# MG-RAST/Shock

Hardware: AMD Instinct MI355X
Metric: device-resident index-build GiB/s + Mrecords/s, 10 GiB FASTQ, 1/2/4/8 GPU (higher is better)
Workload: dtype u8; 1 GPU; fastq record index, 10 GiB synthetic node file in HBM (BASELINE configs[1]); records=30969274, bytes=10737418240, tile=16384, parallelism=single slab, exchange=none (one slab: no collective)

## Files before the change

### shock_amd/csrc/sidx_build.cpp

```cpp
#include <errno.h>
#include <hip/hip_runtime.h>
#include <stdio.h>
#include <stdlib.h>
#include <string.h>
#include <sys/mman.h>
#include <unistd.h>

#include <atomic>
#include <mutex>
#include <vector>

#include "../../include/shockidx.h"
#include "sidx_common.hpp"
#include "sidx_subset.hpp"
#include "sidx_launch.hpp"
#include "sidx_host.hpp"

using namespace sidx;

namespace sidx_host {

CopyPool::CopyPool(int n) : nt_(n) {
  for (int i = 0; i < n; ++i) th_.emplace_back([this, i] { run(i); });
}
CopyPool::~CopyPool() {
  {
    std::lock_guard<std::mutex> g(m_);
    stop_ = true;
    ++gen_;
  }
  cv_.notify_all();
  for (auto &t : th_) t.join();
}
void CopyPool::copy(void *dst, const void *src, size_t n) {
  uint8_t *d = (uint8_t *)dst;
  const uint8_t *sp = (const uint8_t *)src;
  parallel(n, [d, sp](size_t a, size_t b) { memcpy(d + a, sp + a, b - a); });
}
void CopyPool::parallel(size_t n, const std::function<void(size_t, size_t)> &f) {
  if (n < (4u << 20) || nt_ < 2) {
    if (n) f(0, n);
    return;
  }
  std::unique_lock<std::mutex> lk(m_);
  fn_ = &f;
  n_ = n;
  pending_ = nt_;
  ++gen_;
  cv_.notify_all();
  done_.wait(lk, [this] { return pending_ == 0; });
}
void CopyPool::run(int i) {
  unsigned long long seen = 0;
// ... 172 lines not shown
  p.n = n;
  p.end = geom ? geom->end : n;
  p.front = geom ? geom->front : 0;
  p.base = geom ? geom->base : 0;
  p.state_in = geom ? geom->state_in : 0;
  p.row_base = geom ? geom->row_base : 0;
  p.summary = geom ? (u64 *)geom->d_summary : nullptr;
  p.row_cap = row_cap;
  p.rows = d_rows;
  auto status_array = [c](StatusArray a) { return c->d_status + (u64)a * c->tiles_cap(); };
  p.status = status_array(SA_STATUS);
  p.pcnt = status_array(SA_PCNT);
  p.ppre = status_array(SA_PPRE);
  for (int i = 0; i < 2; ++i) p.scan_look[i] = status_array((StatusArray)(SA_LOOK0 + i));
  p.tile_agg = status_array(SA_TILE_AGG);
  p.tile_excl = status_array(SA_TILE_EXCL);
  p.pgrid = c->tiles_grid < ntiles ? c->tiles_grid : (u32)ntiles;
  p.fix = general ? nullptr : c->d_fix.get();
  p.fixcap = (u32)c->tiles_cap();
  p.grid_cap = c->grid_cap;
  p.badkey = (u64 *)(c->d_small + SMALL_BADKEY + 8 * slot);
  p.badkey_next = (u64 *)(c->d_small + SMALL_BADKEY + 8 * (slot ^ 1));
  p.detail = c->d_detail;
  p.counters = (u32 *)(c->d_small + SMALL_COUNTERS + 4 * NCOUNTERS * slot);
  p.counters_next = (u32 *)(c->d_small + SMALL_COUNTERS + 4 * NCOUNTERS * (slot ^ 1));
  p.ntiles = (u32)ntiles;
  p.epoch = c->epoch;
  p.seq = geom ? geom->seq : 0;
  p.inject = (c->inject & 4) ? 1u : 0u;
  p.eof = geom ? geom->eof : 1;
  p.file_start = geom ? geom->file_start : 1;
  p.gate = gate;
  p.gate_fmt = kfmt;
  if (const char *dbg = getenv("SHOCKIDX_DEBUG")) p.debug = (u32)atoi(dbg);
  if (getenv("SHOCKIDX_TIMING")) {
    HIPCHK(hipMemsetAsync(c->d_timing, 0, 9 * 8 * 65536, s), "timing clear");
    p.timing = c->d_timing;
  }
  DevResult *d_res = (DevResult *)(c->d_small + SMALL_RESULT);
  const bool tile_pass = pass != TP_TWO_PASS;
  if (tile_pass) {
    p.tile_stage = c->d_tile_stage;
    p.tile_words = c->d_tile_words;
  }
  p.fq_lines = (pass == TP_FQ && c->want_spans) ? c->d_fqlines.get() : nullptr;
  c->last_spans = false;
  std::unique_lock<std::mutex> device_lock(device_mutex(c->device));
  hipEvent_t k0 = tile_pass ? c->ev0 : c->ek0;
  if (!tile_pass) HIPCHK(hipEventRecord(c->ev0, s), "event");
  static const char *const what[] = {"index launch", "tile pass launch", "FASTA tile pass launch",
                                     "line tile pass launch", "SAM tile pass launch"};
  HIPCHK(sidx_launch_tiles(pass, &p, d_res, s, k0, c->ek1), what[pass]);
  if (res) res->path = tile_pass ? 1u : 2u;
  HIPCHK(hipEventRecord(c->ev1, s), "event");
  if (d_rows && verify_rows()) HIPCHK(sidx_launch_verify_rows(d_rows, p.row_base, row_cap, d_res, s), "verify launch");
  HIPCHK(hipMemcpyAsync(c->h_res, d_res, sizeof(DevResult), hipMemcpyDeviceToHost, s), "result copy");
  HIPCHK(hipStreamSynchronize(s), "index sync");
  c->slots_dirty = false;
  if (p.fq_lines) {
    c->last_p = p;
    c->last_spans = true;
  }
  float ms = 0.f;
  (void)hipEventElapsedTime(&ms, c->ev0, c->ev1);
  if (res) res->kernel_ms += ms;
  float kms = 0.f;
  (void)hipEventElapsedTime(&kms, k0, c->ek1);
  if (res) res->index_ms = kms;
  *dr = *c->h_res;
  device_lock.unlock();
  if ((dr->flags & RF_FIXQUEUE) && !general) {
    if (res) res->reruns++;
    return run_index(c, d_data, n, kfmt, d_rows, row_cap, s, dr, res, geom, true, gate);
  }
  return 0;
}

int translate(shockidx_ctx *c, const DevResult &dr, const uint8_t *d_data, hipStream_t s,
              shockidx_result *res) {
  res->count = dr.count;
  res->fixups = dr.fixups;
  res->fix_tiles = dr.fix_tiles;
  res->state_out = dr.state_out;
  res->term_code = dr.code;
  res->flags = dr.flags;
  if (dr.flags & RF_INTERNAL) return set_msg(res, SHOCKIDX_EINTERNAL, "internal error: device invariant violated");
  if (dr.flags & RF_HALO) return set_msg(res, SHOCKIDX_EINTERNAL, "internal error: slab halo exhausted");
  if (dr.code == ST_OK || dr.code == ST_END || dr.code == ST_ABSENT) {
    res->status = SHOCKIDX_OK;
    return SHOCKIDX_OK;
  }
  if (dr.code == ST_FA_INVALID) {
    return fasta_error_text(res, dr.err_len, [&](char *dst, u64 k) -> int {
      hipError_t e = hipMemcpyAsync(dst, d_data + dr.err_pos, k, hipMemcpyDeviceToHost, s);
      if (e == hipSuccess) e = hipStreamSynchronize(s);
      return e == hipSuccess ? 0 : set_hip(res, e, "error text copy");
    });
  }
  const char *m = status_message(dr.code);
  if (!m) return set_msg(res, SHOCKIDX_EINTERNAL, "internal error: unknown device status");
  return set_msg(res, SHOCKIDX_EFORMAT, m);
}

int build_resident(shockidx_ctx *c, const uint8_t *d_data, u64 n, int kind, int fmt, hipStream_t s,
                   shockidx_result *res) {
  int kfmt = 0;
  const int *gate = nullptr;
  if (int rc = resolve_format(c, d_data, n, kind, fmt, s, &kfmt, res, &gate)) return rc;
  res->format = kfmt == F_LINE ? SHOCKIDX_FMT_LINE : kfmt;
  u64 cap = kfmt == F_LINE ? n / 16 + 4096 : n / 32 + 4096;
  for (int attempt = 0; attempt < 3; ++attempt) {
    if (int rc = c->d_rows.ensure(cap, res)) return rc;
    DevResult dr;
    if (int rc = run_index(c, d_data, n, kfmt, c->d_rows, c->d_rows.cap, s, &dr, res, nullptr, false, gate)) return rc;
    if (gate) {
      gate = nullptr;
      if (int rc = respeculate(c, dr, &kfmt, res)) {
        if (rc < 0 || rc == SHOCKIDX_EFORMAT) return rc;
        res->reruns++;
        continue;
      }
    }
    if (dr.flags & RF_CAPACITY) {
      cap = dr.count;
      res->reruns++;
      continue;
    }
    return translate(c, dr, d_data, s, res);
  }
  return set_msg(res, SHOCKIDX_EINTERNAL, "internal error: row capacity");
}

uint64_t *alloc_rows_out(size_t bytes) {
  constexpr size_t HUGE = 2u << 20;
  if (bytes < 4 * HUGE) return (uint64_t *)malloc(bytes ? bytes : 16);
  void *p = nullptr;
  if (posix_memalign(&p, HUGE, (bytes + HUGE - 1) & ~(HUGE - 1))) return nullptr;
  (void)madvise(p, (bytes + HUGE - 1) & ~(HUGE - 1), MADV_HUGEPAGE);
  return (uint64_t *)p;
}

// ... 194 lines not shown
```

### shock_amd/csrc/sidx_capi.cpp

```cpp
#include <errno.h>
#include <fcntl.h>
#include <hip/hip_runtime.h>
#include <stdio.h>
#include <stdlib.h>
#include <string.h>
#include <unistd.h>

#include <atomic>
#include <random>
#include <string>
#include <thread>

#include <rccl/rccl.h>

#include "../../include/shockidx.h"
#include "sidx_common.hpp"
#include "sidx_subset.hpp"
#include "sidx_launch.hpp"
#include "sidx_slabwalk.hpp"
#include "sidx_host.hpp"

using namespace sidx;
using namespace sidx_host;

// ... 54 lines not shown
  return SHOCKIDX_OK;
}

int shockidx_ctx_create(int device, shockidx_ctx **out) {
  const Err res;
  if (!out) return SHOCKIDX_EINVAL;
  *out = nullptr;
  int ndev = 0;
  HIPCHK(hipGetDeviceCount(&ndev), "hipGetDeviceCount");
  if (device < 0 || device >= ndev) return SHOCKIDX_EINVAL;
  HIPCHK(hipSetDevice(device), "hipSetDevice");
  shockidx_ctx *c = new shockidx_ctx();
  c->device = device;
  hipError_t e = hipStreamCreateWithFlags(&c->stream, hipStreamNonBlocking);
  if (e == hipSuccess) e = hipEventCreate(&c->ev0);
  if (e == hipSuccess) e = hipEventCreate(&c->ev1);
  if (e == hipSuccess) e = hipEventCreate(&c->ek0);
  if (e == hipSuccess) e = hipEventCreate(&c->ek1);
  for (int i = 0; i < NSTAGE && e == hipSuccess; ++i) e = hipEventCreateWithFlags(&c->stage_ev[i], hipEventDisableTiming);
  if (e == hipSuccess) e = hipMalloc(&c->d_small, SMALL_BYTES);
  if (e == hipSuccess) e = hipMemsetAsync(c->d_small, 0, SMALL_BYTES, c->stream);
  if (e == hipSuccess) e = hipMemsetAsync(c->d_small + SMALL_BADKEY, 0xFF, 16, c->stream);
  if (e == hipSuccess) e = hipStreamSynchronize(c->stream);
  if (e == hipSuccess) {
    int cus = 0;
    e = hipDeviceGetAttribute(&cus, hipDeviceAttributeMultiprocessorCount, device);
    int pp = sidx_tiles_blocks_per_cu();
    if (const char *w = getenv("SHOCKIDX_TILES_PER_CU")) pp = atoi(w) < pp ? atoi(w) : pp;
    c->tiles_grid = (u32)(cus * (pp < 1 ? 1 : pp));
    const int vb = sidx_cr_verify_blocks_per_cu();
    c->cr_grid = (u32)(cus * (vb < 1 ? 1 : vb));
  }
  for (int i = 0; i < NSTAGE && e == hipSuccess; ++i) e = hipHostMalloc(&c->h_stage[i], STAGE_BYTES, 0);
  if (e == hipSuccess) e = hipHostMalloc(&c->h_res, sizeof(DevResult), 0);
  if (e == hipSuccess) e = hipHostMalloc(&c->h_det, 64, 0);
  if (e == hipSuccess) {
    const unsigned hw = std::thread::hardware_concurrency();
    int nt = getenv("SHOCKIDX_COPY_THREADS") ? atoi(getenv("SHOCKIDX_COPY_THREADS")) : (int)(hw / 2 < 16 ? hw / 2 : 16);
    c->pool = new CopyPool(nt < 1 ? 1 : nt);
  }
  if (const char *cap = getenv("SHOCKIDX_WORKSPACE_CAP")) c->ws_cap = strtoull(cap, nullptr, 10);
  if (const char *cap = getenv("SHOCKIDX_DEV_CAP")) c->dev_cap = parse_bytes(cap);
  if (e != hipSuccess) {
    shockidx_ctx_destroy(c);
    return SHOCKIDX_EHIP;
  }
  *out = c;
  return SHOCKIDX_OK;
}

int shockidx_ctx_set_dev_cap(shockidx_ctx *c, uint64_t bytes) {
  if (!c) return SHOCKIDX_EINVAL;
  c->dev_cap = bytes;
  return SHOCKIDX_OK;
}

int shockidx_ctx_trim(shockidx_ctx *c, uint64_t keep_bytes) {
  if (!c) return SHOCKIDX_EINVAL;
  if (hipSetDevice(c->device) != hipSuccess) return SHOCKIDX_EHIP;
  trim_workspace(c, keep_bytes);
  return SHOCKIDX_OK;
}

uint64_t shockidx_ctx_workspace_bytes(shockidx_ctx *c) { return c ? workspace_bytes(c) : 0; }

void shockidx_ctx_destroy(shockidx_ctx *c) {
  if (!c) return;
// ... 465 lines not shown
```

### shock_amd/csrc/sidx_common.hpp

```cpp
#pragma once
#include <stdint.h>

namespace sidx {

typedef unsigned long long u64;
typedef long long i64;
typedef unsigned int u32;

#ifndef SIDX_TILE
#define SIDX_TILE 16384
#endif
#ifndef SIDX_NTHREADS
#define SIDX_NTHREADS (SIDX_TILE / 128)
#endif
constexpr int TILE = SIDX_TILE;
constexpr int NTHREADS = SIDX_NTHREADS;
constexpr int NWAVES = NTHREADS / 64;
constexpr int CHUNK = 16;
constexpr int NCHUNKS = TILE / CHUNK;
constexpr int CPT = NCHUNKS / NTHREADS;
constexpr int REGION = TILE / NTHREADS;
constexpr int MAX_DEFER = 16;
constexpr int FQ_TILE_WORDS = 2 * MAX_DEFER;
#ifndef SIDX_HALO
// ... 7 lines not shown

enum Status : u32 {
  ST_OK = 0,
  ST_END = 1,
  ST_FQ_TRUNC = 2,
  ST_FQ_EMPTYLINES = 3,
  ST_FQ_NOAT = 4,
  ST_FQ_NOID = 5,
  ST_FQ_EMPTYSEQ = 6,
  ST_FQ_NOPLUS = 7,
  ST_FQ_IDMISMATCH = 8,
  ST_FQ_LENMISMATCH = 9,
  ST_FA_INVALID = 10,
  ST_DONTCARE = 11,
  ST_NEEDMORE = 12,
  ST_ABSENT = 13,
  ST_DEFER = 14,
  ST_SLOW = 15,
};

constexpr u64 FLAG_AGG = 1ull << 62;
constexpr u64 FLAG_INC = 2ull << 62;
constexpr int EPOCH_SHIFT = 48;
constexpr u32 EPOCH_MASK = 0x3FFF;
constexpr u64 PAYLOAD_MASK = (1ull << EPOCH_SHIFT) - 1;

constexpr int KEY_TILE_BITS = 24;
constexpr int KEY_REC_SHIFT = 4 + KEY_TILE_BITS;
constexpr u64 KEY_NONE = ~0ull;
constexpr int NCOUNTERS = 8;

enum TilePass : int { TP_TWO_PASS = 0, TP_FQ, TP_FA, TP_LINE, TP_SAM };

struct SlabParams {
  const uint8_t *data;
  u64 n;
  u64 end;
  u64 base;
  u64 state_in;
  u64 row_base;
  u64 row_cap;
  u64 *rows;
  u64 *status;
  u64 *badkey;
  u64 *detail;
  u32 *counters;
  u64 *badkey_next;
  u32 *counters_next;
  u32 ntiles;
  u32 epoch;
  int eof;
  int file_start;
  u64 *timing;
  u64 *summary;
  u64 front;
  u32 debug;
  u64 *pcnt;
  u64 *ppre;
  u64 *scan_look[2];
  u32 pgrid;
  u32 seq;
  u64 *fix;
  u32 fixcap;
  u32 grid_cap;
  const u64 *tile_excl;
  u64 *tile_agg;
  u32 *tile_stage;
  u32 *tile_words;
  const int *gate;
  int gate_fmt;
  u32 inject;
  uint16_t *fq_lines;
};

struct SlabSummary {
  u64 agg, state_in, key, natural, row_base, err_pos, err_len;
  uint16_t fmt, flags;
  u32 seq;
};
static_assert(sizeof(SlabSummary) == 64, "summary is exchanged as 64 bytes");

struct SlabPlan {
  u64 state_in, first_record, count, err_pos, err_len;
  u32 code;
  int err_rank;
  u32 inconsistent, flags;
};

constexpr u32 RF_CAPACITY = 1;
constexpr u32 RF_INTERNAL = 2;
constexpr u32 RF_HALO = 4;
constexpr u32 RF_FIXQUEUE = 8;
constexpr u32 RF_MISSPEC = 16;

struct ColKey {
  u64 off, lo, len;
};
enum ColCtl : int { COL_BAD = 0, COL_NB, COL_B, COL_CTL_WORDS };
constexpr u64 COL_KEYCAP = 64ull << 10;
enum ColSlabCtl : int { COLS_MORE = COL_CTL_WORDS, COLS_LAST, COLS_KLO, COLS_KLEN, COLS_ROWS, COL_SLAB_WORDS };
static_assert(COL_SLAB_WORDS == 8, "the host reads the control words through 64 pinned bytes");
struct ColCarryHalf {
  u64 prev_cut, rows, seen, klen;
  uint8_t key[COL_KEYCAP];
};
// ... 30 lines not shown
```

### shock_amd/csrc/sidx_host.hpp

```cpp
#pragma once
#include <hip/hip_runtime.h>
#include <stdint.h>
#include <string.h>

#include <chrono>
#include <condition_variable>
#include <functional>
#include <mutex>
#include <string>
#include <thread>
#include <vector>

#include "../../include/shockidx.h"
#include "sidx_common.hpp"
#include "sidx_devbuf.hpp"

namespace sidx_host {

constexpr size_t STAGE_BYTES = 64ull << 20;
constexpr int NSTAGE = 2;
constexpr size_t SMALL_BADKEY = 0, SMALL_COUNTERS = 64, SMALL_RESULT = 128, SMALL_DETECT = 320, SMALL_CHUNK = 384,
                 SMALL_SLABSUM = 448, SMALL_BYTES = 512;
enum StatusArray : int { SA_STATUS, SA_PCNT, SA_PPRE, SA_LOOK0, SA_LOOK1, SA_TILE_AGG, SA_TILE_EXCL, STATUS_ARRAYS };

// ... 23 lines not shown

}

namespace sidx_host {
hipError_t dev_malloc(void **p, size_t bytes, bool node);
const DevAlloc *hip_allocator();
}

struct shockidx_ctx {
  typedef sidx::u64 u64;
  typedef sidx::u32 u32;
  template <class T, size_t PER = 1> using Buf = sidx_host::DevBuf<T, PER>;
  typedef sidx_host::BufClass BufClass;
  int device = 0;
  hipStream_t stream = nullptr;
  hipEvent_t ev0 = nullptr, ev1 = nullptr, ek0 = nullptr, ek1 = nullptr;
  hipEvent_t stage_ev[sidx_host::NSTAGE] = {nullptr, nullptr};
  sidx_host::BufSet bufs{sidx_host::hip_allocator()};
  Buf<uint8_t> d_in{bufs, BufClass::Large, true};
  Buf<u64, 2> d_rows{bufs};
  Buf<u64> d_status{bufs, BufClass::Tile, false, "hipMalloc(status)"};
  Buf<u64> d_detail{bufs, BufClass::Tile, false, "hipMalloc(detail)"};
  Buf<u64> d_fix{bufs, BufClass::Tile, false, "hipMalloc(fix)"};
  u64 tiles_cap() const { return d_fix.cap / 4; }
  uint8_t *d_small = nullptr;
  u32 epoch = 0;
  bool slots_dirty = false;
  int spec_fmt = 0;
  u64 *d_timing = nullptr;
  u32 tiles_grid = 0;
  u32 grid_cap = 0;
  uint8_t *h_stage[sidx_host::NSTAGE] = {nullptr, nullptr};
  sidx::DevResult *h_res = nullptr;
  sidx_host::CopyPool *pool = nullptr;
  Buf<uint8_t> d_sub{bufs};
  int *h_det = nullptr;
  u64 ws_cap = 0;
  u64 dev_cap = 0;
  Buf<u32> d_tile_stage{bufs};
  Buf<u32> d_tile_words{bufs};
  Buf<uint8_t> d_cra{bufs};
  Buf<uint8_t> d_crb{bufs};
  Buf<uint8_t> d_slot[2] = {Buf<uint8_t>{bufs, BufClass::Large, true, "hipMalloc(slab slot)"},
                            Buf<uint8_t>{bufs, BufClass::Large, true, "hipMalloc(slab slot)"}};
  u32 cr_grid = 0;
  Buf<uint8_t> d_cola{bufs};
  Buf<uint8_t> d_colb{bufs};
  Buf<uint8_t> d_plan{bufs};
  Buf<uint8_t> d_sec{bufs};
  shockidx_stream_stats stream_stats = {};
  Buf<uint8_t> d_batch{bufs};
  Buf<uint8_t> d_bnodes{bufs};
  shockidx_batch_stats batch_stats = {};
  hipStream_t s_copy = nullptr;
  uint8_t *h_rows[2] = {nullptr, nullptr};
  bool want_spans = false;
  Buf<uint16_t> d_fqlines{bufs};
  sidx::SlabParams last_p;
  bool last_spans = false;
  u32 inject = 0;
};

namespace sidx_host {

int set_hip(Err r, hipError_t e, const char *what);
template <class R> void reset_result(R *r) {
// ... 129 lines not shown
```

### shock_amd/csrc/sidx_kernels.hip

```cpp
#include <hip/hip_runtime.h>
#include <hip/hip_ext.h>
#include <atomic>

#include "sidx_claim.hpp"
#include "sidx_common.hpp"
#include "sidx_device.hpp"
#include "sidx_launch.hpp"
#include "sidx_stage.hpp"
#include "sidx_validate.hpp"

namespace sidx {

#ifndef SIDX_DIAG
#define SIDX_DIAG 0
#endif
__device__ __forceinline__ u32 dbg(const SlabParams &p) { return SIDX_DIAG ? p.debug : 0u; }
__device__ __forceinline__ u64 *tmg(const SlabParams &p) { return SIDX_DIAG ? p.timing : nullptr; }

template <int F> struct Traits;
template <> struct Traits<F_FASTQ> { typedef CountMonoid M; static constexpr bool kX = false; static constexpr u32 xc = 0; };
template <> struct Traits<F_LINE>  { typedef CountMonoid M; static constexpr bool kX = false; static constexpr u32 xc = 0; };
template <> struct Traits<F_FASTA> { typedef FastaMonoid M; static constexpr bool kX = true; static constexpr u32 xc = '>'; };
template <> struct Traits<F_SAM>   { typedef SamMonoid M;   static constexpr bool kX = true; static constexpr u32 xc = '@'; };

// ... 2104 lines not shown
        if (pend != ~0ull && lane == 0) put_row(p, pk, pend, g - pend);
        ++cnt;
        pend = g;
        pk = cnt;
        armed = false;
      }
      lo = g + 1;
      pos = g + 1;
    }
    if (bad) continue;
    if (pend != ~0ull) {
      const u64 e = fa_next_global(p, t + 1, lane);
      if (e == p.n && p.end > p.n) fa_halo_close(p, pend, pk, p.fixcap + i, lane);
      else if (lane == 0) put_row(p, pk, pend, e - pend);
    }
    if (t == p.ntiles - 1 && p.eof && p.end == p.n && cnt != s0) {
      bool ok = true;
      u64 q;
      if (p.n - lo > 1 && wa.find(C_NL, lo, p.n, q) == FR_FOUND) fasta_piece_ok(wa, lo, p.n, ok);
      if (!ok) fa_report(p, cnt, (u32)t, lo, p.n - lo, lane);
    }
  }
  if (res) last_block_finalize(p, F_FASTA, res);
}

template <class M>
__device__ __forceinline__ u64 apply_fmt(u64 s, u64 a) { return M::apply(s, a); }

__device__ __forceinline__ void finalize_body(const SlabParams &p, int fmt, DevResult *res);
__global__ void k_finalize(const SlabParams p, int fmt, DevResult *res) {
  if (threadIdx.x != 0 || blockIdx.x != 0) return;
  finalize_body(p, fmt, res);
}
__device__ __forceinline__ void finalize_body(const SlabParams &p, int fmt, DevResult *res) {
  if (gated_off(p)) {
    DevResult r = {};
    r.flags = RF_MISSPEC;
    r.fmt = (u32)fmt;
    r.detected = (u32)*p.gate;
    *res = r;
    *p.badkey_next = KEY_NONE;
    for (int i = 0; i < NCOUNTERS; ++i) p.counters_next[i] = 0;
    return;
  }
  const u64 w = ((volatile u64 *)p.status)[p.ntiles - 1];
  const u64 agg = w & PAYLOAD_MASK;
  u64 fin;
  if (fmt == F_FASTA) fin = apply_fmt<FastaMonoid>(p.state_in, agg);
  else if (fmt == F_SAM) fin = apply_fmt<SamMonoid>(p.state_in, agg);
  else fin = apply_fmt<CountMonoid>(p.state_in, agg);
  const u64 key = __hip_atomic_load(p.badkey, __ATOMIC_RELAXED, __HIP_MEMORY_SCOPE_AGENT);
  DevResult r;
  r.state_out = fin;
  r.slab_agg = agg;
  r.err_pos = 0;
  r.err_len = 0;
  r.flags = 0;
  r.path = 0;
  r.fixups = p.counters[2];
  r.fix_tiles = p.counters[3] >> 1;
  r.fmt = (u32)fmt;
  r.detected = p.gate ? (u32)*p.gate : 0u;
  r.pad = 0;
  r.key = key;
  if ((w >> 62) != 2 || (((u32)(w >> EPOCH_SHIFT)) & EPOCH_MASK) != p.epoch) r.flags |= RF_INTERNAL;
  u64 krec = key >> KEY_REC_SHIFT;
  u32 kst = (u32)(key & 15);
  const u32 ktile = (u32)((key >> 4) & ((1u << KEY_TILE_BITS) - 1));
  const u64 natural = natural_count(fmt, fin);
  r.natural = natural;
  if (key == KEY_NONE) {
    r.count = natural;
    r.code = ST_OK;
  } else {
    r.count = krec;
    r.code = kst;
    if (kst == ST_FA_INVALID) {
      r.err_pos = p.detail[2 * (u64)ktile];
      r.err_len = p.detail[2 * (u64)ktile + 1];
    }
    if (kst == ST_DONTCARE) r.flags |= RF_INTERNAL;
    if (kst == ST_NEEDMORE) r.flags |= RF_HALO;
  }
  if (p.counters[1]) r.flags |= RF_INTERNAL;
  if (p.counters[3] & 1) r.flags |= RF_FIXQUEUE;
  if (p.inject & 1) r.count = r.count ? r.count - 1 : 0;
  const u64 nrows = r.count > p.row_base ? r.count - p.row_base : 0;
  if (nrows > p.row_cap) r.flags |= RF_CAPACITY;
  if (p.file_start && p.eof && p.end == p.n && !(r.flags & (RF_CAPACITY | RF_FIXQUEUE)) && nrows && p.rows) {
    const u64 *rw = p.rows;
    bool bad = rw[0] != p.base;
    if (r.code == ST_OK || r.code == ST_END || r.code == ST_ABSENT) {
      const u64 e = rw[2 * (nrows - 1)] + rw[2 * (nrows - 1) + 1], fe = p.base + p.n;
      if (fmt == F_FASTQ) bad |= e > fe || (e < fe && (p.data[e - p.base] != '\n' || p.data[p.n - 1] != '\n'));
      else bad |= e != fe;
      if (fmt == F_LINE) bad |= rw[2 * (nrows - 1) + 1] != 0 && p.n && p.data[p.n - 1] == '\n';
    }
    if (bad) r.flags |= RF_INTERNAL;
  }
  *res = r;
  if (p.summary) {
    SlabSummary *o = reinterpret_cast<SlabSummary *>(p.summary);
    o->agg = agg; o->state_in = p.state_in; o->key = key; o->natural = natural;
    o->row_base = p.row_base; o->err_pos = r.err_pos; o->err_len = r.err_len;
    o->fmt = (uint16_t)fmt; o->flags = (uint16_t)r.flags; o->seq = p.seq;
  }
  *p.badkey_next = KEY_NONE;
  for (int i = 0; i < NCOUNTERS; ++i) p.counters_next[i] = 0;
}

constexpr int SCAN_T = 256, SCAN_ITEMS = 8, SCAN_BLOCK = SCAN_T * SCAN_ITEMS;

template <class M>
__global__ __launch_bounds__(SCAN_T) void k_scan_excl(const u64 *agg, u64 *excl, u32 n, u64 *look, u32 *ticket,
                                                      u64 *total_word, u32 epoch, u64 in_mask, const int *gate,
                                                      int gate_fmt) {
  __shared__ u64 wtot[SCAN_T / 64];
  __shared__ u64 bpre;
  __shared__ u32 sbid;
  if (gate && *gate != gate_fmt) return;
  const int tid = threadIdx.x, lane = tid & 63, wid = tid >> 6;
  if (tid == 0) sbid = __hip_atomic_fetch_add((gu32 *)ticket, 1u, __ATOMIC_RELAXED, __HIP_MEMORY_SCOPE_AGENT);
  __syncthreads();
  const u32 bid = sbid;
  const u64 i0 = (u64)bid * SCAN_BLOCK + (u64)tid * SCAN_ITEMS;
  u64 v[SCAN_ITEMS];
#pragma unroll
  for (int k = 0; k < SCAN_ITEMS; ++k) v[k] = (i0 + k < n) ? (agg[i0 + k] & in_mask) : M::identity();
#pragma unroll
  for (int k = 1; k < SCAN_ITEMS; ++k) v[k] = M::combine(v[k - 1], v[k]);
  const u64 tinc = wave_incl_scan<M>(v[SCAN_ITEMS - 1], lane);
  u64 texc = __shfl_up(tinc, 1, 64);
  if (lane == 0) texc = M::identity();
// ... 62 lines not shown
  return hipOccupancyMaxActiveBlocksPerMultiprocessor(&n, kern, SNT, 0) == hipSuccess && n > 0 ? n : 1;
}
u32 tile_grid(const SlabParams &p, TilePass pass) {
  static std::atomic<int> occ[TP_SAM + 1], cus[64];
  int dev = 0;
  (void)hipGetDevice(&dev);
  std::atomic<int> &cu_slot = cus[dev & 63];
  int cu = cu_slot.load(std::memory_order_relaxed);
  if (!cu) {
    (void)hipDeviceGetAttribute(&cu, hipDeviceAttributeMultiprocessorCount, dev);
    cu_slot.store(cu, std::memory_order_relaxed);
  }
  int oc = occ[pass].load(std::memory_order_relaxed);
  if (!oc) {
    oc = pass == TP_FA ? occupancy(k_fa_tiles) : pass == TP_SAM ? occupancy(k_sam_tiles) : occupancy(k_line_tiles);
    occ[pass].store(oc, std::memory_order_relaxed);
  }
  const u64 g = (u64)(cu > 0 ? cu : 1) * (u64)(oc > 0 ? oc : 1);
  return (u32)(g < p.ntiles ? g : p.ntiles);
}
u32 place_grid(u64 ntiles, u64 per) {
  const u64 g = (ntiles + per - 1) / per;
  return (u32)(g < 65536 ? g : 65536);
}
template <class M>
hipError_t scan_excl(const SlabParams &p, const u64 *agg, u64 *excl, int which, bool total, hipStream_t s,
                     u64 in_mask = ~0ull) {
  const u32 nb = (p.ntiles + SCAN_BLOCK - 1) / SCAN_BLOCK;
  hipLaunchKernelGGL(k_scan_excl<M>, dim3(nb ? nb : 1), dim3(SCAN_T), 0, s, agg, excl, p.ntiles,
                     p.scan_look[which], p.counters + 4 + which, total ? p.status + (p.ntiles - 1) : p.scan_look[which] + nb,
                     p.epoch, in_mask, p.gate, p.gate_fmt);
  return hipGetLastError();
}
hipError_t finalize(const SlabParams &p, int fmt, DevResult *d_res, hipStream_t s) {
  hipError_t e = hipGetLastError();
  if (e != hipSuccess) return e;
  hipLaunchKernelGGL(k_finalize, dim3(1), dim3(64), 0, s, p, fmt, d_res);
  return hipGetLastError();
}

template <int F>
hipError_t launch_two_pass(const SlabParams &p, DevResult *d_res, hipStream_t s, hipEvent_t ek0, hipEvent_t ek1) {
  const dim3 g1(p.ntiles), block(NTHREADS);
  if (ek0) (void)hipEventRecord(ek0, s);
  hipLaunchKernelGGL(k_tile_agg<F>, g1, block, 0, s, p, p.tile_agg);
  hipError_t e = scan_excl<typename Traits<F>::M>(p, p.tile_agg, (u64 *)p.tile_excl, 0, true, s);
  if (e != hipSuccess) return e;
  hipLaunchKernelGGL(k_index1<F>, g1, block, 0, s, p);
  e = hipGetLastError();
  if (e != hipSuccess) return e;
  if (ek1) (void)hipEventRecord(ek1, s);
  return finalize(p, F, d_res, s);
}

constexpr u32 FIX_GRID = 64;
hipError_t launch_fq(const SlabParams &p, DevResult *d_res, hipStream_t s, hipEvent_t ek0, hipEvent_t ek1) {
  if (p.fq_lines) hipExtLaunchKernelGGL(k_fq_tiles<true>, dim3(p.pgrid), dim3(SNT), 0, s, ek0, ek1, 0, p);
  else hipExtLaunchKernelGGL(k_fq_tiles<false>, dim3(p.pgrid), dim3(SNT), 0, s, ek0, ek1, 0, p);
  hipError_t e = scan_excl<CountMonoid>(p, p.tile_agg, (u64 *)p.tile_excl, 0, true, s, FQW_TMASK);
  if (e != hipSuccess) return e;
  if (p.debug & 4096u) return hipErrorLaunchFailure;
  hipLaunchKernelGGL(k_fq_place, dim3(place_grid(p.ntiles, PLACE_TILES)), dim3(256), 0, s, p);
  hipLaunchKernelGGL(k_fixup, dim3(FIX_GRID), dim3(256), 0, s, p, d_res);
  return hipGetLastError();
}

hipError_t launch_fa(const SlabParams &p, DevResult *d_res, hipStream_t s, hipEvent_t ek0, hipEvent_t ek1) {
  hipExtLaunchKernelGGL(k_fa_tiles, dim3(p.pgrid), dim3(SNT), 0, s, ek0, ek1, 0, p);
  hipError_t e = scan_excl<FastaMonoid>(p, p.tile_agg, (u64 *)p.tile_excl, 0, true, s, FAW_AMASK);
  if (e != hipSuccess) return e;
  hipLaunchKernelGGL(k_fa_place, dim3(place_grid(p.ntiles, PLACE_TILES)), dim3(256), 0, s, p);
  hipLaunchKernelGGL(k_fa_fixup, dim3(FIX_GRID), dim3(256), 0, s, p, d_res);
  return hipGetLastError();
}

hipError_t launch_line(const SlabParams &p, DevResult *d_res, hipStream_t s, hipEvent_t ek0, hipEvent_t ek1) {
  hipExtLaunchKernelGGL(k_line_tiles, dim3(p.pgrid), dim3(SNT), 0, s, ek0, ek1, 0, p);
  hipError_t e = scan_excl<CountMonoid>(p, p.tile_agg, (u64 *)p.tile_excl, 0, true, s, LCOUNT);
  if (e == hipSuccess) e = scan_excl<MaxMonoid>(p, p.pcnt, p.ppre, 1, false, s);
  if (e != hipSuccess) return e;
  hipLaunchKernelGGL(k_line_place<F_LINE>, dim3(place_grid(p.ntiles, LPLACE_TILES)), dim3(256), 0, s, p);
  hipLaunchKernelGGL(k_line_final, dim3(1), dim3(64), 0, s, p);
  return finalize(p, F_LINE, d_res, s);
}

hipError_t launch_sam(const SlabParams &p, DevResult *d_res, hipStream_t s, hipEvent_t ek0, hipEvent_t ek1) {
  hipExtLaunchKernelGGL(k_sam_tiles, dim3(p.pgrid), dim3(SNT), 0, s, ek0, ek1, 0, p);
  hipError_t e = scan_excl<SamMonoid>(p, p.tile_agg, (u64 *)p.tile_excl, 0, true, s);
  if (e != hipSuccess) return e;
  hipLaunchKernelGGL(k_sam_resolve, dim3((p.ntiles + 255) / 256), dim3(256), 0, s, p);
  e = scan_excl<MaxMonoid>(p, p.pcnt, p.ppre, 1, false, s);
  if (e != hipSuccess) return e;
  hipLaunchKernelGGL(k_line_place<F_SAM>, dim3(place_grid(p.ntiles, LPLACE_TILES)), dim3(256), 0, s, p);
  hipLaunchKernelGGL(k_sam_final, dim3(1), dim3(64), 0, s, p);
  return finalize(p, F_SAM, d_res, s);
}
}

extern "C" hipError_t sidx_launch_tiles(TilePass pass, const SlabParams *pp, DevResult *d_res, hipStream_t s,
                                        hipEvent_t ek0, hipEvent_t ek1) {
  SlabParams p = *pp;
  if (pass == TP_FA || pass == TP_LINE || pass == TP_SAM) p.pgrid = tile_grid(p, pass);
  if (p.grid_cap && p.pgrid > p.grid_cap) p.pgrid = p.grid_cap;
  switch (pass) {
    case TP_FQ: return launch_fq(p, d_res, s, ek0, ek1);
    case TP_FA: return launch_fa(p, d_res, s, ek0, ek1);
    case TP_LINE: return launch_line(p, d_res, s, ek0, ek1);
    case TP_SAM: return launch_sam(p, d_res, s, ek0, ek1);
    case TP_TWO_PASS:
      switch (p.gate_fmt) {
        case F_FASTQ: return launch_two_pass<F_FASTQ>(p, d_res, s, ek0, ek1);
        case F_FASTA: return launch_two_pass<F_FASTA>(p, d_res, s, ek0, ek1);
        case F_SAM: return launch_two_pass<F_SAM>(p, d_res, s, ek0, ek1);
        case F_LINE: return launch_two_pass<F_LINE>(p, d_res, s, ek0, ek1);
      }
  }
  return hipErrorInvalidValue;
}

static_assert(FQ_LINE_E + FQ_OVF <= 2 * RCAP, "a FASTQ tile's starts fit its slot");
extern "C" u64 sidx_tile_stage_words(TilePass pass, u64 ntiles, u32 grid) {
  return (pass == TP_LINE || pass == TP_SAM) ? ntiles * (LCAP / 2) : (ntiles + grid + 16) * (u64)RCAP;
}

extern "C" hipError_t sidx_launch_fq_spans_place(const SlabParams *pp, u32 *spans, u64 *outlen, u64 K, int kind,
                                                hipStream_t s) {
  const SlabParams &p = *pp;
  if (!p.fq_lines || !p.ntiles) return hipSuccess;
  hipLaunchKernelGGL(k_fq_spans_place, dim3(place_grid(p.ntiles, 4)), dim3(256), 0, s, p, spans, outlen, K, kind);
  return hipGetLastError();
}

extern "C" int sidx_tiles_blocks_per_cu() {
  int n = 0;
  return hipOccupancyMaxActiveBlocksPerMultiprocessor(&n, k_fq_tiles<false>, SNT, 0) == hipSuccess ? n : 0;
}
```

### shock_amd/csrc/sidx_launch.hpp

```cpp
#pragma once
#include <hip/hip_runtime.h>
#include <stddef.h>
#include <stdint.h>

#include "sidx_batch.hpp"
#include "sidx_common.hpp"

extern "C" {

hipError_t sidx_launch_detect(const uint8_t *d, sidx::u64 n, int *d_out, hipStream_t s);
hipError_t sidx_launch_detect_sections(const uint8_t *d, sidx::u64 n, const void *d_secs, sidx::u64 nsecs, int *d_out,
    hipStream_t s);
hipError_t sidx_launch_tiles(sidx::TilePass pass, const sidx::SlabParams *p, sidx::DevResult *d_res, hipStream_t s,
    hipEvent_t ek0, hipEvent_t ek1);
sidx::u64 sidx_tile_stage_words(sidx::TilePass pass, sidx::u64 ntiles, sidx::u32 grid);
hipError_t sidx_launch_chunkrecord(const uint8_t *d, sidx::u64 n, int fasta, long long chunk, sidx::u64 *rows,
    sidx::u64 row_cap, sidx::u64 *out, long long curr0, sidx::u64 cnt0, sidx::u64 max_steps, hipStream_t s);
hipError_t sidx_cr_gpos_count(const uint8_t *d, sidx::u64 n, sidx::u64 *tcnt, sidx::u64 *toff, uint16_t *slot,
    void *scan_tmp, size_t *scan_bytes, hipStream_t s);
hipError_t sidx_cr_gpos_write(const uint8_t *d, sidx::u64 n, const sidx::u64 *tcnt, const sidx::u64 *toff,
    const uint16_t *slot, sidx::u64 *G, hipStream_t s);
sidx::u32 sidx_cr_gslot();
hipError_t sidx_cr_graph(const uint8_t *d, sidx::u64 n, int fasta, sidx::u64 chunk, const sidx::u64 *base,
    sidx::u64 stride, sidx::u64 count, sidx::u64 *ft, sidx::u32 *J1, sidx::u32 *Ja, sidx::u32 *Jb, int levels,
    const sidx::u32 **JL, hipStream_t s);
hipError_t sidx_cr_round(const uint8_t *d, sidx::u64 n, int fasta, sidx::u64 chunk, const sidx::u64 *base,
    sidx::u64 stride, sidx::u64 count, const sidx::u64 *ft, const sidx::u32 *JL, const sidx::u32 *J1, sidx::u32 L,
    sidx::u64 y, sidx::u64 k0, sidx::u64 cap, sidx::u32 *heads, sidx::u64 *pos, sidx::i64 *mres, sidx::u64 *ctl,
    sidx::u64 *rows, sidx::u64 row_cap, sidx::u32 verify_grid, hipStream_t s);
int sidx_cr_verify_blocks_per_cu();
sidx::u32 sidx_fa_slot();
hipError_t sidx_fa_bnd_count(const uint8_t *d, sidx::u64 n, sidx::u64 *lnl, sidx::u64 *lgt, sidx::u64 *cnl,
    sidx::u64 *cgt, sidx::u64 *tcnt, sidx::u64 *toff, uint16_t *slot, void *tmp, size_t *tmp_bytes, hipStream_t s);
hipError_t sidx_fa_bnd_write(const uint8_t *d, sidx::u64 n, const sidx::u64 *cnl, const sidx::u64 *cgt,
    const sidx::u64 *tcnt, const sidx::u64 *toff, const uint16_t *slot, sidx::u64 *B, hipStream_t s);
hipError_t sidx_fa_anon_spans(const uint8_t *d, sidx::u64 n, const sidx::u64 *B, sidx::u64 bstride, sidx::u64 m,
    sidx::u64 *bspan, sidx::u64 *outlen, sidx::u64 *firstbad, hipStream_t s);
hipError_t sidx_fa_anon_write(const uint8_t *d, sidx::u64 n, const sidx::u64 *bspan, const sidx::u64 *outoff,
    sidx::u64 K, uint8_t *out, hipStream_t s);
hipError_t sidx_sam_anon_spans(const uint8_t *d, sidx::u64 n, const sidx::u64 *rows, sidx::u64 K, sidx::u64 *span,
    sidx::u64 *outlen, sidx::u64 *firstbad, sidx::u64 *firsteof, hipStream_t s);
hipError_t sidx_sam_anon_write(const uint8_t *d, const sidx::u64 *span, const sidx::u64 *outlen,
    const sidx::u64 *outoff, sidx::u64 K, uint8_t *out, sidx::u64 *count, hipStream_t s);
hipError_t sidx_crs_scan(const sidx::u64 *ri, sidx::u64 R, sidx::u64 *len, sidx::u64 *P, void *tmp,
    size_t *scan_bytes, hipStream_t s);
hipError_t sidx_crs_build(const sidx::u64 *P, sidx::u64 R, sidx::u32 *J1, sidx::u32 *Ja, sidx::u32 *Jb, int levels,
    sidx::u32 *heads, sidx::u64 *rows, sidx::u64 row_cap, sidx::u64 *ctl, hipStream_t s);
// ... 100 lines not shown
```

Baseline: 4783 GiB/s.

## Write build result to mapped host memory and spin-wait instead of stream sync

The finalize/fixup kernel now writes the DevResult directly into coherent mapped pinned host memory, then stores an epoch tag with system scope. The host polls that tag with a bounded spin before confirming with an event query, instead of doing a D2H memcpy plus hipStreamSynchronize. The end event is folded into the last kernel launch via hipExtLaunchKernelGGL, which drops a separate event record. The aim is to cut sync and copy latency at the end of each build, at the cost of CPU spinning and reliance on correct device-to-host memory ordering.

New measurement: 4800 GiB/s (median of 6 runs). No clear change (+0.4%).

```diff
diff --git a/shock_amd/csrc/sidx_build.cpp b/shock_amd/csrc/sidx_build.cpp
--- a/shock_amd/csrc/sidx_build.cpp
+++ b/shock_amd/csrc/sidx_build.cpp
@@ -18,7 +18,40 @@
 
 using namespace sidx;
 
+#ifndef SIDX_DIAG
+#define SIDX_DIAG 0
+#endif
+
 namespace sidx_host {
+
+static bool stamps_on() { return SIDX_DIAG && getenv("SHOCKIDX_STAMPS"); }
+
+constexpr double SPIN_MS = 200.0, QUERY_MS = 1.0;
+static inline void cpu_relax() {
+#if defined(__x86_64__) || defined(__i386__)
+  __builtin_ia32_pause();
+#endif
+}
+static hipError_t wait_build(shockidx_ctx *c, hipStream_t s, u32 tag) {
+  if (const char *w = getenv("SHOCKIDX_WAIT")) {
+    if (!strcmp(w, "stream")) return hipStreamSynchronize(s);
+    if (!strcmp(w, "event")) return hipEventSynchronize(c->ev1);
+  }
+  const u32 *word = &c->h_res->pad;
+  const double t0 = now_ms();
+  for (u32 i = 0; __atomic_load_n(word, __ATOMIC_ACQUIRE) != tag; ++i) {
+    cpu_relax();
+    if ((i & 4095u) == 4095u && now_ms() - t0 > SPIN_MS) return hipStreamSynchronize(s);
+  }
+  const double t1 = now_ms();
+  for (u32 i = 0;; ++i) {
+    const hipError_t e = hipEventQuery(c->ev1);
+    if (e != hipErrorNotReady) return e;
+    if ((i & 15u) == 15u && now_ms() - t1 > QUERY_MS) break;
+  }
+  (void)hipGetLastError();
+  return hipEventSynchronize(c->ev1);
+}
 
 CopyPool::CopyPool(int n) : nt_(n) {
   for (int i = 0; i < n; ++i) th_.emplace_back([this, i] { run(i); });
@@ -257,6 +290,7 @@
   p.file_start = geom ? geom->file_start : 1;
   p.gate = gate;
   p.gate_fmt = kfmt;
+  p.host_res = c->d_hres;
   if (const char *dbg = getenv("SHOCKIDX_DEBUG")) p.debug = (u32)atoi(dbg);
   if (getenv("SHOCKIDX_TIMING")) {
     HIPCHK(hipMemsetAsync(c->d_timing, 0, 9 * 8 * 65536, s), "timing clear");
@@ -275,12 +309,19 @@
   if (!tile_pass) HIPCHK(hipEventRecord(c->ev0, s), "event");
   static const char *const what[] = {"index launch", "tile pass launch", "FASTA tile pass launch",
                                      "line tile pass launch", "SAM tile pass launch"};
-  HIPCHK(sidx_launch_tiles(pass, &p, d_res, s, k0, c->ek1), what[pass]);
+  c->h_res->pad = 0;
+  const double t_launch = stamps_on() ? now_ms() : 0.0;
+  HIPCHK(sidx_launch_tiles(pass, &p, d_res, s, k0, c->ek1, c->ev1), what[pass]);
+  const double t_launched = stamps_on() ? now_ms() : 0.0;
   if (res) res->path = tile_pass ? 1u : 2u;
-  HIPCHK(hipEventRecord(c->ev1, s), "event");
-  if (d_rows && verify_rows()) HIPCHK(sidx_launch_verify_rows(d_rows, p.row_base, row_cap, d_res, s), "verify launch");
-  HIPCHK(hipMemcpyAsync(c->h_res, d_res, sizeof(DevResult), hipMemcpyDeviceToHost, s), "result copy");
-  HIPCHK(hipStreamSynchronize(s), "index sync");
+  if (d_rows && verify_rows()) {
+    HIPCHK(sidx_launch_verify_rows(d_rows, p.row_base, row_cap, d_res, s), "verify launch");
+    HIPCHK(hipMemcpyAsync(c->h_res, d_res, sizeof(DevResult), hipMemcpyDeviceToHost, s), "result copy");
+    HIPCHK(hipStreamSynchronize(s), "index sync");
+  } else {
+    HIPCHK(wait_build(c, s, p.epoch), "index sync");
+  }
+  const double t_waited = stamps_on() ? now_ms() : 0.0;
   c->slots_dirty = false;
   if (p.fq_lines) {
     c->last_p = p;
@@ -292,7 +333,11 @@
   float kms = 0.f;
   (void)hipEventElapsedTime(&kms, k0, c->ek1);
   if (res) res->index_ms = kms;
+  if (stamps_on())
+    fprintf(stderr, "{\"stamp\": \"run_index\", \"n\": %llu, \"launch_ms\": %.4f, \"wait_ms\": %.4f, \"submit_to_return_ms\": %.4f, "
+            "\"kernel_ms\": %.4f, \"index_ms\": %.4f}\n", n, t_launched - t_launch, t_waited - t_launched, t_waited - t_launch, ms, kms);
   *dr = *c->h_res;
+  dr->pad = 0;
   device_lock.unlock();
   if ((dr->flags & RF_FIXQUEUE) && !general) {
     if (res) res->reruns++;
@@ -331,7 +376,9 @@
                    shockidx_result *res) {
   int kfmt = 0;
   const int *gate = nullptr;
+  const double t_fmt = stamps_on() ? now_ms() : 0.0;
   if (int rc = resolve_format(c, d_data, n, kind, fmt, s, &kfmt, res, &gate)) return rc;
+  if (stamps_on()) fprintf(stderr, "{\"stamp\": \"resolve_format\", \"ms\": %.4f}\n", now_ms() - t_fmt);
   res->format = kfmt == F_LINE ? SHOCKIDX_FMT_LINE : kfmt;
   u64 cap = kfmt == F_LINE ? n / 16 + 4096 : n / 32 + 4096;
   for (int attempt = 0; attempt < 3; ++attempt) {
diff --git a/shock_amd/csrc/sidx_capi.cpp b/shock_amd/csrc/sidx_capi.cpp
--- a/shock_amd/csrc/sidx_capi.cpp
+++ b/shock_amd/csrc/sidx_capi.cpp
@@ -110,7 +110,8 @@
     c->cr_grid = (u32)(cus * (vb < 1 ? 1 : vb));
   }
   for (int i = 0; i < NSTAGE && e == hipSuccess; ++i) e = hipHostMalloc(&c->h_stage[i], STAGE_BYTES, 0);
-  if (e == hipSuccess) e = hipHostMalloc(&c->h_res, sizeof(DevResult), 0);
+  if (e == hipSuccess) e = hipHostMalloc(&c->h_res, sizeof(DevResult), hipHostMallocMapped | hipHostMallocCoherent);
+  if (e == hipSuccess) e = hipHostGetDevicePointer((void **)&c->d_hres, c->h_res, 0);
   if (e == hipSuccess) e = hipHostMalloc(&c->h_det, 64, 0);
   if (e == hipSuccess) {
     const unsigned hw = std::thread::hardware_concurrency();
diff --git a/shock_amd/csrc/sidx_common.hpp b/shock_amd/csrc/sidx_common.hpp
--- a/shock_amd/csrc/sidx_common.hpp
+++ b/shock_amd/csrc/sidx_common.hpp
@@ -63,6 +63,8 @@
 
 enum TilePass : int { TP_TWO_PASS = 0, TP_FQ, TP_FA, TP_LINE, TP_SAM };
 
+struct DevResult;
+
 struct SlabParams {
   const uint8_t *data;
   u64 n;
@@ -102,6 +104,7 @@
   int gate_fmt;
   u32 inject;
   uint16_t *fq_lines;
+  DevResult *host_res;
 };
 
 struct SlabSummary {
diff --git a/shock_amd/csrc/sidx_host.hpp b/shock_amd/csrc/sidx_host.hpp
--- a/shock_amd/csrc/sidx_host.hpp
+++ b/shock_amd/csrc/sidx_host.hpp
@@ -79,6 +79,7 @@
   u32 grid_cap = 0;
   uint8_t *h_stage[sidx_host::NSTAGE] = {nullptr, nullptr};
   sidx::DevResult *h_res = nullptr;
+  sidx::DevResult *d_hres = nullptr;
   sidx_host::CopyPool *pool = nullptr;
   Buf<uint8_t> d_sub{bufs};
   int *h_det = nullptr;
diff --git a/shock_amd/csrc/sidx_kernels.hip b/shock_amd/csrc/sidx_kernels.hip
--- a/shock_amd/csrc/sidx_kernels.hip
+++ b/shock_amd/csrc/sidx_kernels.hip
@@ -2160,13 +2160,22 @@
   if (threadIdx.x != 0 || blockIdx.x != 0) return;
   finalize_body(p, fmt, res);
 }
+__device__ __forceinline__ void put_result(const SlabParams &p, DevResult *res, const DevResult &r) {
+  *res = r;
+  if (p.host_res) {
+    *p.host_res = r;
+    __builtin_amdgcn_fence(__ATOMIC_RELEASE, "");
+    asm volatile("s_waitcnt vmcnt(0)" ::: "memory");
+    __hip_atomic_store(&p.host_res->pad, p.epoch, __ATOMIC_RELAXED, __HIP_MEMORY_SCOPE_SYSTEM);
+  }
+}
 __device__ __forceinline__ void finalize_body(const SlabParams &p, int fmt, DevResult *res) {
   if (gated_off(p)) {
     DevResult r = {};
     r.flags = RF_MISSPEC;
     r.fmt = (u32)fmt;
     r.detected = (u32)*p.gate;
-    *res = r;
+    put_result(p, res, r);
     *p.badkey_next = KEY_NONE;
     for (int i = 0; i < NCOUNTERS; ++i) p.counters_next[i] = 0;
     return;
@@ -2226,7 +2235,7 @@
     }
     if (bad) r.flags |= RF_INTERNAL;
   }
-  *res = r;
+  put_result(p, res, r);
   if (p.summary) {
     SlabSummary *o = reinterpret_cast<SlabSummary *>(p.summary);
     o->agg = agg; o->state_in = p.state_in; o->key = key; o->natural = natural;
@@ -2355,15 +2364,16 @@
                      p.epoch, in_mask, p.gate, p.gate_fmt);
   return hipGetLastError();
 }
-hipError_t finalize(const SlabParams &p, int fmt, DevResult *d_res, hipStream_t s) {
+hipError_t finalize(const SlabParams &p, int fmt, DevResult *d_res, hipStream_t s, hipEvent_t ev_end) {
   hipError_t e = hipGetLastError();
   if (e != hipSuccess) return e;
-  hipLaunchKernelGGL(k_finalize, dim3(1), dim3(64), 0, s, p, fmt, d_res);
+  hipExtLaunchKernelGGL(k_finalize, dim3(1), dim3(64), 0, s, nullptr, ev_end, 0, p, fmt, d_res);
   return hipGetLastError();
 }
 
 template <int F>
-hipError_t launch_two_pass(const SlabParams &p, DevResult *d_res, hipStream_t s, hipEvent_t ek0, hipEvent_t ek1) {
+hipError_t launch_two_pass(const SlabParams &p, DevResult *d_res, hipStream_t s, hipEvent_t ek0, hipEvent_t ek1,
+                     hipEvent_t ev_end) {
   const dim3 g1(p.ntiles), block(NTHREADS);
   if (ek0) (void)hipEventRecord(ek0, s);
   hipLaunchKernelGGL(k_tile_agg<F>, g1, block, 0, s, p, p.tile_agg);
@@ -2373,41 +2383,45 @@
   e = hipGetLastError();
   if (e != hipSuccess) return e;
   if (ek1) (void)hipEventRecord(ek1, s);
-  return finalize(p, F, d_res, s);
+  return finalize(p, F, d_res, s, ev_end);
 }
 
 constexpr u32 FIX_GRID = 64;
-hipError_t launch_fq(const SlabParams &p, DevResult *d_res, hipStream_t s, hipEvent_t ek0, hipEvent_t ek1) {
+hipError_t launch_fq(const SlabParams &p, DevResult *d_res, hipStream_t s, hipEvent_t ek0, hipEvent_t ek1,
+                     hipEvent_t ev_end) {
   if (p.fq_lines) hipExtLaunchKernelGGL(k_fq_tiles<true>, dim3(p.pgrid), dim3(SNT), 0, s, ek0, ek1, 0, p);
   else hipExtLaunchKernelGGL(k_fq_tiles<false>, dim3(p.pgrid), dim3(SNT), 0, s, ek0, ek1, 0, p);
   hipError_t e = scan_excl<CountMonoid>(p, p.tile_agg, (u64 *)p.tile_excl, 0, true, s, FQW_TMASK);
   if (e != hipSuccess) return e;
   if (p.debug & 4096u) return hipErrorLaunchFailure;
   hipLaunchKernelGGL(k_fq_place, dim3(place_grid(p.ntiles, PLACE_TILES)), dim3(256), 0, s, p);
-  hipLaunchKernelGGL(k_fixup, dim3(FIX_GRID), dim3(256), 0, s, p, d_res);
+  hipExtLaunchKernelGGL(k_fixup, dim3(FIX_GRID), dim3(256), 0, s, nullptr, ev_end, 0, p, d_res);
   return hipGetLastError();
 }
 
-hipError_t launch_fa(const SlabParams &p, DevResult *d_res, hipStream_t s, hipEvent_t ek0, hipEvent_t ek1) {
+hipError_t launch_fa(const SlabParams &p, DevResult *d_res, hipStream_t s, hipEvent_t ek0, hipEvent_t ek1,
+                     hipEvent_t ev_end) {
   hipExtLaunchKernelGGL(k_fa_tiles, dim3(p.pgrid), dim3(SNT), 0, s, ek0, ek1, 0, p);
   hipError_t e = scan_excl<FastaMonoid>(p, p.tile_agg, (u64 *)p.tile_excl, 0, true, s, FAW_AMASK);
   if (e != hipSuccess) return e;
   hipLaunchKernelGGL(k_fa_place, dim3(place_grid(p.ntiles, PLACE_TILES)), dim3(256), 0, s, p);
-  hipLaunchKernelGGL(k_fa_fixup, dim3(FIX_GRID), dim3(256), 0, s, p, d_res);
+  hipExtLaunchKernelGGL(k_fa_fixup, dim3(FIX_GRID), dim3(256), 0, s, nullptr, ev_end, 0, p, d_res);
   return hipGetLastError();
 }
 
-hipError_t launch_line(const SlabParams &p, DevResult *d_res, hipStream_t s, hipEvent_t ek0, hipEvent_t ek1) {
+hipError_t launch_line(const SlabParams &p, DevResult *d_res, hipStream_t s, hipEvent_t ek0, hipEvent_t ek1,
+                     hipEvent_t ev_end) {
   hipExtLaunchKernelGGL(k_line_tiles, dim3(p.pgrid), dim3(SNT), 0, s, ek0, ek1, 0, p);
   hipError_t e = scan_excl<CountMonoid>(p, p.tile_agg, (u64 *)p.tile_excl, 0, true, s, LCOUNT);
   if (e == hipSuccess) e = scan_excl<MaxMonoid>(p, p.pcnt, p.ppre, 1, false, s);
   if (e != hipSuccess) return e;
   hipLaunchKernelGGL(k_line_place<F_LINE>, dim3(place_grid(p.ntiles, LPLACE_TILES)), dim3(256), 0, s, p);
   hipLaunchKernelGGL(k_line_final, dim3(1), dim3(64), 0, s, p);
-  return finalize(p, F_LINE, d_res, s);
-}
-
-hipError_t launch_sam(const SlabParams &p, DevResult *d_res, hipStream_t s, hipEvent_t ek0, hipEvent_t ek1) {
+  return finalize(p, F_LINE, d_res, s, ev_end);
+}
+
+hipError_t launch_sam(const SlabParams &p, DevResult *d_res, hipStream_t s, hipEvent_t ek0, hipEvent_t ek1,
+                     hipEvent_t ev_end) {
   hipExtLaunchKernelGGL(k_sam_tiles, dim3(p.pgrid), dim3(SNT), 0, s, ek0, ek1, 0, p);
   hipError_t e = scan_excl<SamMonoid>(p, p.tile_agg, (u64 *)p.tile_excl, 0, true, s);
   if (e != hipSuccess) return e;
@@ -2416,26 +2430,26 @@
   if (e != hipSuccess) return e;
   hipLaunchKernelGGL(k_line_place<F_SAM>, dim3(place_grid(p.ntiles, LPLACE_TILES)), dim3(256), 0, s, p);
   hipLaunchKernelGGL(k_sam_final, dim3(1), dim3(64), 0, s, p);
-  return finalize(p, F_SAM, d_res, s);
+  return finalize(p, F_SAM, d_res, s, ev_end);
 }
 }
 
 extern "C" hipError_t sidx_launch_tiles(TilePass pass, const SlabParams *pp, DevResult *d_res, hipStream_t s,
-                                        hipEvent_t ek0, hipEvent_t ek1) {
+                                        hipEvent_t ek0, hipEvent_t ek1, hipEvent_t ev_end) {
   SlabParams p = *pp;
   if (pass == TP_FA || pass == TP_LINE || pass == TP_SAM) p.pgrid = tile_grid(p, pass);
   if (p.grid_cap && p.pgrid > p.grid_cap) p.pgrid = p.grid_cap;
   switch (pass) {
-    case TP_FQ: return launch_fq(p, d_res, s, ek0, ek1);
-    case TP_FA: return launch_fa(p, d_res, s, ek0, ek1);
-    case TP_LINE: return launch_line(p, d_res, s, ek0, ek1);
-    case TP_SAM: return launch_sam(p, d_res, s, ek0, ek1);
+    case TP_FQ: return launch_fq(p, d_res, s, ek0, ek1, ev_end);
+    case TP_FA: return launch_fa(p, d_res, s, ek0, ek1, ev_end);
+    case TP_LINE: return launch_line(p, d_res, s, ek0, ek1, ev_end);
+    case TP_SAM: return launch_sam(p, d_res, s, ek0, ek1, ev_end);
     case TP_TWO_PASS:
       switch (p.gate_fmt) {
-        case F_FASTQ: return launch_two_pass<F_FASTQ>(p, d_res, s, ek0, ek1);
-        case F_FASTA: return launch_two_pass<F_FASTA>(p, d_res, s, ek0, ek1);
-        case F_SAM: return launch_two_pass<F_SAM>(p, d_res, s, ek0, ek1);
-        case F_LINE: return launch_two_pass<F_LINE>(p, d_res, s, ek0, ek1);
+        case F_FASTQ: return launch_two_pass<F_FASTQ>(p, d_res, s, ek0, ek1, ev_end);
+        case F_FASTA: return launch_two_pass<F_FASTA>(p, d_res, s, ek0, ek1, ev_end);
+        case F_SAM: return launch_two_pass<F_SAM>(p, d_res, s, ek0, ek1, ev_end);
+        case F_LINE: return launch_two_pass<F_LINE>(p, d_res, s, ek0, ek1, ev_end);
       }
   }
   return hipErrorInvalidValue;
diff --git a/shock_amd/csrc/sidx_launch.hpp b/shock_amd/csrc/sidx_launch.hpp
--- a/shock_amd/csrc/sidx_launch.hpp
+++ b/shock_amd/csrc/sidx_launch.hpp
@@ -12,7 +12,7 @@
 hipError_t sidx_launch_detect_sections(const uint8_t *d, sidx::u64 n, const void *d_secs, sidx::u64 nsecs, int *d_out,
     hipStream_t s);
 hipError_t sidx_launch_tiles(sidx::TilePass pass, const sidx::SlabParams *p, sidx::DevResult *d_res, hipStream_t s,
-    hipEvent_t ek0, hipEvent_t ek1);
+    hipEvent_t ek0, hipEvent_t ek1, hipEvent_t ev_end);
 sidx::u64 sidx_tile_stage_words(sidx::TilePass pass, sidx::u64 ntiles, sidx::u32 grid);
 hipError_t sidx_launch_chunkrecord(const uint8_t *d, sidx::u64 n, int fasta, long long chunk, sidx::u64 *rows,
     sidx::u64 row_cap, sidx::u64 *out, long long curr0, sidx::u64 cnt0, sidx::u64 max_steps, hipStream_t s);
```
